# WU-CVGL/Styl3R

Hardware: AMD Instinct MI355X
Metric: 256x256 stylized views/sec (fwd+bwd) @ ~65k Gaussians (higher is better)
Workload: dtype f32; 1 GPU; rasterizer fwd+bwd (decoder API + MSE, the loss computed inside the composite kernels): 10 scenes x 4 target views/GPU/step, 256x256, G=65536 Gaussians/scene (1 ctx view x 256x256), sh_degree=0, make_scale_invariant, all views in one batched launch; outputs the decoder discards are not computed (decoder_splatting_cuda.py:37-68 drops radii / opacity / n_touched, MSE sends no depth gradient: the com; parallelism=dp1 (scenes sharded)

## Files before the change

styl3r_amd/csrc/gsr_common.h:

```cpp
#pragma once
#include <hip/hip_runtime.h>
#include <stdint.h>

#include <type_traits>

#include "../../include/gsr.h"

namespace gsr {

constexpr int TILE = GSR_TILE;
constexpr int TILE_PIX = TILE * TILE;
constexpr int WAVE = 64;

struct alignas(16) SplatRec {
    float x, y, depth;
    uint32_t rad_flags;
    float A, B, C, opacity;
    float r, g, b;
    uint32_t ext;
};
constexpr int LDS_TILES_MAX = 4096;
static_assert(sizeof(SplatRec) == 48, "SplatRec must be 48 bytes");

struct alignas(16) QueueRec {
// ... 46 lines not shown
    return GSR_ELAUNCH;
}
inline bool hip_ok(hipError_t e)
{
    if (e == hipSuccess) return true;
    g_last_hip_error = e;
    return false;
}

struct StageTimer {
    GsrProfile *p; int slot; hipStream_t s;
    StageTimer(void *prof, bool fwd, hipStream_t stream, bool resume = false)
        : p(static_cast<GsrProfile *>(prof)), slot(-1), s(stream)
    {
        if (!p) return;
        int &n = fwd ? p->next_fwd : p->next_bwd;
        if (resume) { if (n > 0 && n <= p->max_calls) slot = n - 1; }
        else if (n < p->max_calls) slot = n++;
    }
    void begin(int stage) { if (slot >= 0 && ((p->mask >> stage) & 1u)) (void)hipEventRecord(p->at(slot, stage, 0), s); }
    void end(int stage) { if (slot >= 0 && ((p->mask >> stage) & 1u)) (void)hipEventRecord(p->at(slot, stage, 1), s); }
};

int layout(const GsrDims &d, long long cap, GsrLayout &L);
Ptrs carve(void *base, const GsrLayout &L);
int forward(const GsrDims &d, const GsrView *views, const float *means, const float *cov6, const float *opac,
            const float *shs, long long cap, void *workspace, size_t workspace_bytes, float *image, float *depth,
            float *opacity, int32_t *radii, int32_t *n_touched, int32_t *status, const GsrFused *fx, hipStream_t stream,
            bool composite = true);
int backward(const GsrDims &d, const GsrView *views, const float *means, const float *cov6, const float *shs,
             long long cap, void *workspace, size_t workspace_bytes, const float *dL_dimage, const float *dL_ddepth,
             float *dL_dmeans, float *dL_dcov6, float *dL_dopac, float *dL_dshs, float *dL_dmeans2D, float *dL_dtau,
             const GsrFused *fx, hipStream_t stream);
int k6_blocks_per_cu(int variant);
int test_reduce9(const float *in, float *out, int rounds, int blocks, int variant, hipStream_t stream);
int forward_styles(const GsrDims &d, int S, const GsrView *views, const float *means, const float *cov6, const float *opac,
                   const float *const *shs, long long cap, void *workspace, size_t workspace_bytes, void *extra, size_t extra_bytes,
                   uint32_t *tile_count, float *image, float *depth, float *opacity, int32_t *radii, int32_t *status, hipStream_t stream);

inline size_t align_up(size_t x, size_t a) { return (x + a - 1) / a * a; }

struct Carver {
    void *base;
    size_t off;
    template <class T>
    T *take(size_t count)
    {
        T *p = base ? reinterpret_cast<T *>(static_cast<char *>(base) + off) : nullptr;
        off += align_up(count * sizeof(T), 256);
        return p;
    }
};

template <class F>
inline void with_sh_degree(const GsrDims &d, F &&f)
{
    switch (d.M > 0 ? d.sh_degree : -1) {
        case -1: f(std::integral_constant<int, -1>{}); break;
        case 0: f(std::integral_constant<int, 0>{}); break;
        case 1: f(std::integral_constant<int, 1>{}); break;
        case 2: f(std::integral_constant<int, 2>{}); break;
        case 3: f(std::integral_constant<int, 3>{}); break;
        default: f(std::integral_constant<int, 4>{}); break;
    }
}

__host__ __device__ inline int tiles_x(int W) { return (W + TILE - 1) / TILE; }
__host__ __device__ inline int tiles_y(int H) { return (H + TILE - 1) / TILE; }

constexpr uint32_t SEG_ONE = 1u << 30;
constexpr int CKPT_SLOT_FLOATS = 5 * TILE_PIX;
__host__ __device__ inline uint32_t seg_len(const GsrDims &d)
{
    switch ((d.flags >> GSR_FLAG_SEG_SHIFT) & 7) {
        case 1: return 64u;
        case 2: return 128u;
        case 3: return 192u;
        case 4: return 256u;
        case 5: return 384u;
        case 7: return SEG_ONE;
        default: {
            const long long vt = (long long)d.B * d.Vt * tiles_x(d.W) * tiles_y(d.H);
            return vt >= 4096 ? 256u : (vt >= 1024 ? 128u : 64u);
        }
    }
}
__host__ __device__ inline size_t unit_capacity(size_t VT, long long cap, uint32_t L) { return VT + (size_t)cap / L; }
__host__ __device__ inline size_t ckpt_slots(long long cap, uint32_t L) { return (size_t)cap / L; }

__device__ constexpr float SH_C0 = 0.28209479177387814f;
__device__ constexpr float SH_C1 = 0.4886025119029199f;
__device__ constexpr float SH_C2_0 = 1.0925484305920792f, SH_C2_1 = -1.0925484305920792f, SH_C2_2 = 0.31539156525252005f,
                           SH_C2_3 = -1.0925484305920792f, SH_C2_4 = 0.5462742152960396f;
__device__ constexpr float SH_C3_0 = -0.5900435899266435f, SH_C3_1 = 2.890611442640554f, SH_C3_2 = -0.4570457994644658f,
                           SH_C3_3 = 0.3731763325901154f, SH_C3_4 = -0.4570457994644658f, SH_C3_5 = 1.445305721320277f,
                           SH_C3_6 = -0.5900435899266435f;
__device__ constexpr float SH_C4_0 = 2.5033429417967046f, SH_C4_1 = -1.7701307697799304f, SH_C4_2 = 0.9461746957575601f,
                           SH_C4_3 = -0.6690465435572892f, SH_C4_4 = 0.10578554691520431f, SH_C4_5 = -0.6690465435572892f,
                           SH_C4_6 = 0.47308734787878004f, SH_C4_7 = -1.7701307697799304f, SH_C4_8 = 0.6258357354491761f;

#pragma clang fp contract(off)

__device__ inline void sh_basis(int deg, float x, float y, float z, float *b)
{
    b[0] = SH_C0;
    if (deg < 1) return;
    b[1] = -SH_C1 * y; b[2] = SH_C1 * z; b[3] = -SH_C1 * x;
    if (deg < 2) return;
    float xx = x * x, yy = y * y, zz = z * z, xy = x * y, yz = y * z, xz = x * z;
    b[4] = SH_C2_0 * xy; b[5] = SH_C2_1 * yz; b[6] = SH_C2_2 * (2.0f * zz - xx - yy);
    b[7] = SH_C2_3 * xz; b[8] = SH_C2_4 * (xx - yy);
    if (deg < 3) return;
    b[9] = SH_C3_0 * y * (3.0f * xx - yy);
    b[10] = SH_C3_1 * xy * z;
    b[11] = SH_C3_2 * y * (4.0f * zz - xx - yy);
    b[12] = SH_C3_3 * z * (2.0f * zz - 3.0f * xx - 3.0f * yy);
    b[13] = SH_C3_4 * x * (4.0f * zz - xx - yy);
    b[14] = SH_C3_5 * z * (xx - yy);
    b[15] = SH_C3_6 * x * (xx - 3.0f * yy);
    if (deg < 4) return;
    b[16] = SH_C4_0 * xy * (xx - yy);
    b[17] = SH_C4_1 * yz * (3.0f * xx - yy);
    b[18] = SH_C4_2 * xy * (7.0f * zz - 1.0f);
    b[19] = SH_C4_3 * yz * (7.0f * zz - 3.0f);
    b[20] = SH_C4_4 * (zz * (35.0f * zz - 30.0f) + 3.0f);
    b[21] = SH_C4_5 * xz * (7.0f * zz - 3.0f);
    b[22] = SH_C4_6 * (xx - yy) * (7.0f * zz - 1.0f);
    b[23] = SH_C4_7 * xz * (xx - 3.0f * yy);
    b[24] = SH_C4_8 * (xx * (xx - 3.0f * yy) - yy * (3.0f * xx - yy));
}

__device__ inline void sh_basis_grad(int deg, float x, float y, float z, float *dx, float *dy, float *dz)
{
    dx[0] = dy[0] = dz[0] = 0.f;
    if (deg < 1) return;
    dx[1] = 0.f; dy[1] = -SH_C1; dz[1] = 0.f;
    dx[2] = 0.f; dy[2] = 0.f; dz[2] = SH_C1;
    dx[3] = -SH_C1; dy[3] = 0.f; dz[3] = 0.f;
    if (deg < 2) return;
    float xx = x * x, yy = y * y, zz = z * z, xy = x * y, yz = y * z, xz = x * z;
    dx[4] = SH_C2_0 * y; dy[4] = SH_C2_0 * x; dz[4] = 0.f;
    dx[5] = 0.f; dy[5] = SH_C2_1 * z; dz[5] = SH_C2_1 * y;
    dx[6] = SH_C2_2 * (-2.0f * x); dy[6] = SH_C2_2 * (-2.0f * y); dz[6] = SH_C2_2 * (4.0f * z);
    dx[7] = SH_C2_3 * z; dy[7] = 0.f; dz[7] = SH_C2_3 * x;
    dx[8] = SH_C2_4 * (2.0f * x); dy[8] = SH_C2_4 * (-2.0f * y); dz[8] = 0.f;
    if (deg < 3) return;
    dx[9] = SH_C3_0 * (6.0f * xy); dy[9] = SH_C3_0 * (3.0f * xx - 3.0f * yy); dz[9] = 0.f;
    dx[10] = SH_C3_1 * yz; dy[10] = SH_C3_1 * xz; dz[10] = SH_C3_1 * xy;
    dx[11] = SH_C3_2 * (-2.0f * xy); dy[11] = SH_C3_2 * (4.0f * zz - xx - 3.0f * yy); dz[11] = SH_C3_2 * (8.0f * yz);
    dx[12] = SH_C3_3 * (-6.0f * xz); dy[12] = SH_C3_3 * (-6.0f * yz); dz[12] = SH_C3_3 * (6.0f * zz - 3.0f * xx - 3.0f * yy);
    dx[13] = SH_C3_4 * (4.0f * zz - 3.0f * xx - yy); dy[13] = SH_C3_4 * (-2.0f * xy); dz[13] = SH_C3_4 * (8.0f * xz);
    dx[14] = SH_C3_5 * (2.0f * xz); dy[14] = SH_C3_5 * (-2.0f * yz); dz[14] = SH_C3_5 * (xx - yy);
    dx[15] = SH_C3_6 * (3.0f * xx - 3.0f * yy); dy[15] = SH_C3_6 * (-6.0f * xy); dz[15] = 0.f;
    if (deg < 4) return;
    dx[16] = SH_C4_0 * y * (3.0f * xx - yy); dy[16] = SH_C4_0 * x * (xx - 3.0f * yy); dz[16] = 0.f;
    dx[17] = SH_C4_1 * (6.0f * xy * z); dy[17] = SH_C4_1 * z * (3.0f * xx - 3.0f * yy); dz[17] = SH_C4_1 * y * (3.0f * xx - yy);
    dx[18] = SH_C4_2 * y * (7.0f * zz - 1.0f); dy[18] = SH_C4_2 * x * (7.0f * zz - 1.0f); dz[18] = SH_C4_2 * (14.0f * xy * z);
    dx[19] = 0.f; dy[19] = SH_C4_3 * z * (7.0f * zz - 3.0f); dz[19] = SH_C4_3 * y * (21.0f * zz - 3.0f);
    dx[20] = 0.f; dy[20] = 0.f; dz[20] = SH_C4_4 * (140.0f * zz * z - 60.0f * z);
    dx[21] = SH_C4_5 * z * (7.0f * zz - 3.0f); dy[21] = 0.f; dz[21] = SH_C4_5 * x * (21.0f * zz - 3.0f);
    dx[22] = SH_C4_6 * (2.0f * x) * (7.0f * zz - 1.0f); dy[22] = SH_C4_6 * (-2.0f * y) * (7.0f * zz - 1.0f); dz[22] = SH_C4_6 * (xx - yy) * (14.0f * z);
    dx[23] = SH_C4_7 * z * (3.0f * xx - 3.0f * yy); dy[23] = SH_C4_7 * (-6.0f * xy * z); dz[23] = SH_C4_7 * x * (xx - 3.0f * yy);
    dx[24] = SH_C4_8 * (4.0f * xx * x - 12.0f * x * yy); dy[24] = SH_C4_8 * (-12.0f * xx * y + 4.0f * yy * y); dz[24] = 0.f;
}

__device__ __forceinline__ void sh_view_dir(const float *m, const float *campos, float &x, float &y, float &z, float &len)
{
    float dx = m[0] - campos[0], dy = m[1] - campos[1], dz = m[2] - campos[2];
    len = sqrtf(dx * dx + dy * dy + dz * dz);
    x = dx / len; y = dy / len; z = dz / len;
}

template <int DEG>
__device__ __forceinline__ uint32_t sh_colour(float x, float y, float z, const float *__restrict__ sh, float *col)
{
    constexpr int NC = (DEG + 1) * (DEG + 1);
    float bs[NC];
    sh_basis(DEG, x, y, z, bs);
    uint32_t clampbits = 0;
#pragma unroll
    for (int c = 0; c < 3; ++c) {
        float acc = bs[0] * sh[c];
#pragma unroll
        for (int k = 1; k < NC; ++k) acc = acc + bs[k] * sh[3 * k + c];
        acc = acc + 0.5f;
        if (acc < 0.f) clampbits |= (1u << c);
        col[c] = fmaxf(acc, 0.f);
    }
    return clampbits;
}

struct Geom {
    float t[3];
    float txc, tyc;
    bool clampx, clampy;
    float J00, J02, J11, J12;
    float M0[3], M1[3];
    float a, b, c;
};

__device__ inline bool geom_eval(const float *V, float tanfovx, float tanfovy, int W, int H, const float *mean,
                                 const float *S, Geom &g)
{
    float px = mean[0], py = mean[1], pz = mean[2];
#pragma unroll
    for (int c = 0; c < 3; ++c) g.t[c] = px * V[0 + c] + py * V[4 + c] + pz * V[8 + c] + V[12 + c];
    if (g.t[2] <= 0.2f) return false;
    float fx = (float)W / (2.0f * tanfovx);
    float fy = (float)H / (2.0f * tanfovy);
    float limx = 1.3f * tanfovx, limy = 1.3f * tanfovy;
    float tz = g.t[2];
    float txtz = g.t[0] / tz, tytz = g.t[1] / tz;
    float cx = fminf(limx, fmaxf(-limx, txtz));
    float cy = fminf(limy, fmaxf(-limy, tytz));
    g.clampx = (txtz < -limx || txtz > limx);
    g.clampy = (tytz < -limy || tytz > limy);
    g.txc = cx * tz;
    g.tyc = cy * tz;
    g.J00 = fx / tz;
    g.J02 = -(fx * g.txc) / (tz * tz);
    g.J11 = fy / tz;
    g.J12 = -(fy * g.tyc) / (tz * tz);
#pragma unroll
    for (int j = 0; j < 3; ++j) {
        float R0 = V[4 * j + 0], R1 = V[4 * j + 1], R2 = V[4 * j + 2];
        g.M0[j] = g.J00 * R0 + g.J02 * R2;
        g.M1[j] = g.J11 * R1 + g.J12 * R2;
    }
    float v0[3], v1[3];
    v0[0] = S[0] * g.M0[0] + S[1] * g.M0[1] + S[2] * g.M0[2];
    v0[1] = S[1] * g.M0[0] + S[3] * g.M0[1] + S[4] * g.M0[2];
    v0[2] = S[2] * g.M0[0] + S[4] * g.M0[1] + S[5] * g.M0[2];
    v1[0] = S[0] * g.M1[0] + S[1] * g.M1[1] + S[2] * g.M1[2];
    v1[1] = S[1] * g.M1[0] + S[3] * g.M1[1] + S[4] * g.M1[2];
    v1[2] = S[2] * g.M1[0] + S[4] * g.M1[1] + S[5] * g.M1[2];
    g.a = (g.M0[0] * v0[0] + g.M0[1] * v0[1] + g.M0[2] * v0[2]) + 0.3f;
    g.b = g.M1[0] * v0[0] + g.M1[1] * v0[1] + g.M1[2] * v0[2];
    g.c = (g.M1[0] * v1[0] + g.M1[1] * v1[1] + g.M1[2] * v1[2]) + 0.3f;
    return true;
}

__device__ inline void load_cov(const float *__restrict__ cov, size_t sg, bool cov9, float *S)
{
    if (cov9) {
        const float *c = cov + 9 * sg;
        S[0] = c[0]; S[1] = c[1]; S[2] = c[2]; S[3] = c[4]; S[4] = c[5]; S[5] = c[8];
    } else {
        const float *c = cov + 6 * sg;
#pragma unroll
        for (int k = 0; k < 6; ++k) S[k] = c[k];
    }
}

__device__ inline int tile_rect(float px, float py, int rad, int gx, int gy, int &minx, int &miny, int &maxx, int &maxy)
{
    minx = min(gx, max(0, (int)((px - (float)rad) / (float)TILE)));
    miny = min(gy, max(0, (int)((py - (float)rad) / (float)TILE)));
    maxx = min(gx, max(0, (int)((px + (float)rad + (float)(TILE - 1)) / (float)TILE)));
    maxy = min(gy, max(0, (int)((py + (float)rad + (float)(TILE - 1)) / (float)TILE)));
    return (maxx - minx) * (maxy - miny);
}

#pragma clang fp contract(fast)

__device__ inline uint32_t quadrant_mask(const float4 q0, const float4 q1, uint32_t ext, int ox, int oy)
{
    uint32_t quad = 0;
    if (ext) {
        const float hx = (float)(ext & 0xffffu), hy = (float)(ext >> 16);
        const float fox = (float)ox - q0.x, foy = (float)oy - q0.y;
        const float A = q1.x, B = q1.y, C = q1.z;
        const float lim = 2.0f * __logf(255.0f * q1.w) * 1.002f + 1e-3f;
#pragma unroll
        for (int k = 0; k < 4; ++k) {
            const float x0 = fox + (float)((k & 1) * 8), x1 = x0 + 7.f;
            const float y0 = foy + (float)((k >> 1) * 8), y1 = y0 + 7.f;
            if (x0 > hx || x1 < -hx || y0 > hy || y1 < -hy) continue;
            float best = 0.f;
            if (!(x0 <= 0.f && x1 >= 0.f && y0 <= 0.f && y1 >= 0.f)) {
                best = 3.0e38f;
                const float iC = -B * __builtin_amdgcn_rcpf(C), iA = -B * __builtin_amdgcn_rcpf(A);
#pragma unroll
                for (int e = 0; e < 2; ++e) {
                    const float xe = e ? x1 : x0;
                    const float dy = fminf(fmaxf(iC * xe, y0), y1);
                    best = fminf(best, A * xe * xe + 2.f * B * xe * dy + C * dy * dy);
                    const float ye = e ? y1 : y0;
                    const float dx = fminf(fmaxf(iA * ye, x0), x1);
                    best = fminf(best, A * dx * dx + 2.f * B * dx * ye + C * ye * ye);
                }
            }
            if (best <= lim) quad |= 1u << k;
        }
    }
    return quad;
}

#define CONIC_PRESCALE 1.4426950408889634f
__device__ inline float footprint_exp(float power) { return __builtin_amdgcn_exp2f(power); }
__device__ inline uint32_t stage_entry_fwd(const SplatRec *__restrict__ recs, uint32_t id, int ox, int oy, float4 *dst)
{
    const float4 *r = reinterpret_cast<const float4 *>(recs + id);
    const float4 q0 = r[0], q1 = r[1], q2 = r[2];
    const uint32_t quad = quadrant_mask(q0, q1, __float_as_uint(q2.w), ox, oy);
    dst[0] = make_float4(q0.x, q0.y, q1.x * CONIC_PRESCALE, q1.y * CONIC_PRESCALE);
    dst[1] = make_float4(q1.z * CONIC_PRESCALE, q1.w, q0.z, __uint_as_float(id));
    dst[2] = make_float4(q2.x, q2.y, q2.z, __uint_as_float(quad));
    return quad;
}
__device__ inline void stage_entry_bwd(const SplatRec *__restrict__ recs, uint32_t id, uint32_t quad, float4 *dst)
{
    const float4 *r = reinterpret_cast<const float4 *>(recs + id);
    const float4 q0 = r[0], q1 = r[1], q2 = r[2];
    dst[0] = make_float4(q0.x, q0.y, q1.x * CONIC_PRESCALE, q1.y * CONIC_PRESCALE);
    dst[1] = make_float4(q1.z * CONIC_PRESCALE, q1.w, q0.z, __uint_as_float(id));
    dst[2] = make_float4(q2.x, q2.y, q2.z, __uint_as_float(quad));
}

__device__ inline float sel_f(unsigned long long m, float t, float f)
{
    float r;
    asm("v_cndmask_b32 %0, %1, %2, %3" : "=v"(r) : "v"(f), "v"(t), "s"(m));
    return r;
}
__device__ inline float sel0_f(unsigned long long m, float t)
{
    float r;
    asm("v_cndmask_b32 %0, 0, %1, %2" : "=v"(r) : "v"(t), "s"(m));
    return r;
}
__device__ inline uint32_t sel_u(unsigned long long m, uint32_t t, uint32_t f)
{
    uint32_t r;
    asm("v_cndmask_b32 %0, %1, %2, %3" : "=v"(r) : "v"(f), "v"(t), "s"(m));
    return r;
}

template <int CTRL, int ROW_MASK = 0xf, int BANK_MASK = 0xf, bool BOUND = false>
__device__ inline float dpp_mov(float v)
{
    return __builtin_bit_cast(float, __builtin_amdgcn_update_dpp(0, __builtin_bit_cast(int, v), CTRL, ROW_MASK, BANK_MASK, BOUND));
}

__device__ inline float wave_sum_to_lane63(float v)
{
    v += dpp_mov<0xb1, 0xf, 0xf, true>(v);
    v += dpp_mov<0x4e, 0xf, 0xf, true>(v);
    v += dpp_mov<0x124, 0xf, 0xf, true>(v);
    v += dpp_mov<0x128, 0xf, 0xf, true>(v);
    v += dpp_mov<0x142, 0xa, 0xf, false>(v);
    v += dpp_mov<0x143, 0xc, 0xf, false>(v);
    return v;
}

__device__ inline double wave_sum(double v)
{
#pragma unroll
    for (int o = 32; o > 0; o >>= 1) v += __shfl_xor(v, o, 64);
    return v;
}

template <bool SLOT>
__device__ inline uint32_t wave_agg_inc(uint32_t *__restrict__ counters, uint32_t t, bool valid)
{
    const int lane = threadIdx.x & 63;
    unsigned long long todo = __ballot(valid);
    int my_leader = lane;
    uint32_t cnt = 0, rank = 0;
    while (todo) {
        const int leader = __ffsll((long long)todo) - 1;
        const uint32_t tl = (uint32_t)__builtin_amdgcn_readlane((int)t, leader);
        const bool mine = valid && t == tl;
        const unsigned long long m = __ballot(mine);
        if (mine) {
            my_leader = leader;
            cnt = (uint32_t)__popcll(m);
            rank = (uint32_t)__popcll(m & ((1ull << lane) - 1ull));
        }
        todo &= ~m;
    }
    uint32_t base = 0;
    if (valid && lane == my_leader) {
        if (SLOT) base = atomicAdd(counters + t, cnt);
        else atomicAdd(counters + t, cnt);
    }
    if (!SLOT) return 0;
    base = (uint32_t)__shfl((int)base, my_leader, 64);
    return base + rank;
}

__device__ inline float row_allsum(float v)
{
    v += dpp_mov<0xb1, 0xf, 0xf, true>(v);
    v += dpp_mov<0x4e, 0xf, 0xf, true>(v);
    v += dpp_mov<0x124, 0xf, 0xf, true>(v);
    v += dpp_mov<0x128, 0xf, 0xf, true>(v);
    return v;
}
__device__ inline float swapsum32(float x, float y)
{
    const auto r = __builtin_amdgcn_permlane32_swap(__float_as_uint(x), __float_as_uint(y), false, false);
    return __uint_as_float(r[0]) + __uint_as_float(r[1]);
}
__device__ inline float swapsum16(float x, float y)
{
    const auto r = __builtin_amdgcn_permlane16_swap(__float_as_uint(x), __float_as_uint(y), false, false);
    return __uint_as_float(r[0]) + __uint_as_float(r[1]);
}
__device__ inline float rows_packed_sum(float x, float y, float u, const bool u_whole_wave)
{
    float z, u8;
    asm volatile("s_nop 1\n\t"
                 "v_add_f32_dpp %0, %2, %2 row_ror:8 row_mask:0xf bank_mask:0x3\n\t"
                 "v_add_f32_dpp %0, %3, %3 row_ror:8 row_mask:0xf bank_mask:0xc\n\t"
                 "v_add_f32_dpp %1, %4, %4 row_ror:8 row_mask:0xf bank_mask:0xf\n\t"
                 "s_nop 0\n\t"
                 "v_add_f32_dpp %0, %0, %0 row_ror:12 row_mask:0xf bank_mask:0x5\n\t"
                 "v_add_f32_dpp %0, %1, %1 row_ror:12 row_mask:0xf bank_mask:0x8\n\t"
                 "s_nop 1\n\t"
                 "v_add_f32_dpp %0, %0, %0 quad_perm:[1,0,3,2] row_mask:0xf bank_mask:0xf\n\t"
                 "s_nop 1\n\t"
                 "v_add_f32_dpp %0, %0, %0 quad_perm:[2,3,0,1] row_mask:0xf bank_mask:0xf"
                 : "=&v"(z), "=&v"(u8) : "v"(x), "v"(y), "v"(u));
    if (u_whole_wave)
        asm volatile("s_nop 1\n\t"
                     "v_add_f32_dpp %0, %0, %0 row_bcast:15 row_mask:0xa bank_mask:0x8\n\t"
                     "s_nop 1\n\t"
                     "v_add_f32_dpp %0, %0, %0 row_bcast:31 row_mask:0xc bank_mask:0x8" : "+v"(z));
    return z;
}
__device__ inline float wave_reduce10(const float *a)
{
    const float b0 = swapsum32(a[0], a[5]), b1 = swapsum32(a[1], a[6]), b2 = swapsum32(a[2], a[7]), b3 = swapsum32(a[3], a[8]),
                b4 = swapsum32(a[4], a[9]);
    return rows_packed_sum(swapsum16(b0, b1), swapsum16(b2, b3), swapsum16(b4, 0.f), false);
}
__device__ inline int reduce10_slot(int lane)
{
    const int r = lane >> 4, s = lane & 15;
    if (s == 0) return (r < 2) ? r : r + 3;
    if (s == 8) return (r < 2) ? r + 2 : r + 5;
    if (s == 12) return (r == 0) ? 4 : (r == 2 ? 9 : -1);
    return -1;
}
__device__ inline float wave_reduce9(const float *v)
{
    const float b0 = swapsum32(v[0], v[4]), b1 = swapsum32(v[1], v[5]), b2 = swapsum32(v[2], v[6]), b3 = swapsum32(v[3], v[7]);
    return rows_packed_sum(swapsum16(b0, b1), swapsum16(b2, b3), v[8], true);
}
__device__ inline int reduce9_slot(int lane)
{
    const int r = lane >> 4, s = lane & 15;
    if (s == 0) return (r < 2) ? r : r + 2;
    if (s == 8) return (r < 2) ? r + 2 : r + 4;
    return lane == 63 ? 8 : -1;
}
__device__ inline float wave_reduce9_lds(const float *v, float *s_red, int lane)
{
#pragma unroll
    for (int i = 0; i < 8; ++i) s_red[i * 64 + lane] = v[i];
    asm volatile("" ::: "memory");
    const float4 p = reinterpret_cast<const float4 *>(s_red)[lane], q = reinterpret_cast<const float4 *>(s_red)[64 + lane];
    asm volatile("" ::: "memory");
    return rows_packed_sum((p.x + p.y) + (p.z + p.w), (q.x + q.y) + (q.z + q.w), v[8], true);
}
__device__ inline int reduce9_lds_slot(int lane)
{
    const int r = lane >> 4, s = lane & 15;
    if (s == 0) return r;
    if (s == 8) return r + 4;
    return lane == 63 ? 8 : -1;
}

}
```

styl3r_amd/csrc/gsr_forward.hip:

```cpp
#include <cstdlib>
#include <cstring>
#include <type_traits>

#include "gsr_common.h"

namespace gsr {

#pragma clang fp contract(off)
template <int DEG>
__global__ void __launch_bounds__(256) k_preprocess(GsrDims d, const GsrView *__restrict__ views,
                                                    const float *__restrict__ means, const float *__restrict__ cov6,
                                                    const float *__restrict__ opac, const float *__restrict__ shs,
                                                    Ptrs ws, int32_t *__restrict__ radii, int lds_tiles)
{
    extern __shared__ uint32_t s_tiles[];
    const int g = blockIdx.x * blockDim.x + threadIdx.x;
    const int b = blockIdx.y;
    const bool live = g < d.G;
    const size_t sg = (size_t)b * d.G + (live ? g : 0);
    const float m0[3] = {means[3 * sg], means[3 * sg + 1], means[3 * sg + 2]};
    float S0[6];
    load_cov(cov6, sg, (d.flags & GSR_FLAG_COV9) != 0, S0);
    const float op = opac[sg];
    if (live) ws.opac[sg] = op;
// ... 265 lines not shown
    }
    uint32_t ftotal;
    const uint32_t fpos = t.full_base + block_excl_scan_256<uint32_t>(unit ? nf : 0u, s4, ftotal);
    if (i >= n) return;
    ws.tile_order[s_base[cls] + atomicAdd(&s_cnt[cls], 1u)] = (uint32_t)i;
    if (!unit) return;
    for (uint32_t s = 0; s < nf; ++s)
        if (fpos + s < umax) ws.unit_order[fpos + s] = make_uint2((uint32_t)i, s);
    const uint32_t p = t.full + s_base[ucl] + atomicAdd(&s_cnt[ucl], 1u);
    if (p < umax) ws.unit_order[p] = make_uint2((uint32_t)i, nf);
}

#pragma clang fp contract(off)
__global__ void __launch_bounds__(256) k_scatter(GsrDims d, Ptrs ws)
{
    if (ws.status[GSR_ST_OVERFLOW]) return;
    const int g = blockIdx.x * blockDim.x + threadIdx.x;
    const int v = blockIdx.y;
    const bool live = g < d.G;
    const size_t vg = (size_t)v * d.G + (live ? g : 0);
    const float4 q0 = ws.geo[vg];
    const int rad = live ? (int)(__float_as_uint(q0.w) & 0xffffffu) : 0;
    const int gx = tiles_x(d.W), gy = tiles_y(d.H), T = gx * gy;
    int minx = 0, miny = 0, maxx = 0, maxy = 0;
    if (rad > 0) tile_rect(q0.x, q0.y, rad, gx, gy, minx, miny, maxx, maxy);
    const unsigned long long key = ((unsigned long long)__float_as_uint(q0.z) << 32) | (unsigned)g;
    const size_t tb = (size_t)v * T;
    const int rw = maxx - minx, area = rw * (maxy - miny);
    int amax = area;
#pragma unroll
    for (int o = 32; o > 0; o >>= 1) amax = max(amax, __shfl_xor(amax, o, 64));
    for (int k = 0; k < amax; ++k) {
        const bool has = k < area;
        const int ty = has ? miny + k / rw : 0, tx = has ? minx + k % rw : 0;
        const uint32_t tl = (uint32_t)(ty * gx + tx);
        const uint32_t slot = wave_agg_inc<true>(ws.tile_cursor + tb, tl, has);
        if (has) ws.pairs[ws.tile_offset[tb + tl] + slot] = key;
    }
}
#pragma clang fp contract(fast)

__global__ void __launch_bounds__(256) k_scatter_lds(GsrDims d, Ptrs ws)
{
    if (ws.status[GSR_ST_OVERFLOW]) return;
    extern __shared__ uint32_t s_sc[];
    const int g = blockIdx.x * blockDim.x + threadIdx.x;
    const int v = blockIdx.y;
    const bool live = g < d.G;
    const size_t vg = (size_t)v * d.G + (live ? g : 0);
    const float4 q0 = ws.geo[vg];
    const int rad = live ? (int)(__float_as_uint(q0.w) & 0xffffffu) : 0;
    const int gx = tiles_x(d.W), gy = tiles_y(d.H), T = gx * gy;
    uint32_t *s_cnt = s_sc, *s_base = s_sc + T;
    for (int t = threadIdx.x; t < T; t += 256) s_cnt[t] = 0u;
    int minx = 0, miny = 0, maxx = 0, maxy = 0;
    if (rad > 0) tile_rect(q0.x, q0.y, rad, gx, gy, minx, miny, maxx, maxy);
    const unsigned long long key = ((unsigned long long)__float_as_uint(q0.z) << 32) | (unsigned)g;
    const size_t tb = (size_t)v * T;
    const int rw = maxx - minx, area = rw * (maxy - miny);
    __syncthreads();
    for (int k = 0; k < area; ++k) atomicAdd(&s_cnt[(miny + k / rw) * gx + minx + k % rw], 1u);
    __syncthreads();
    for (int t = threadIdx.x; t < T; t += 256) {
        const uint32_t c = s_cnt[t];
        if (c) { s_base[t] = ws.tile_offset[tb + t] + atomicAdd(ws.tile_cursor + tb + t, c); s_cnt[t] = 0u; }
    }
    __syncthreads();
    for (int k = 0; k < area; ++k) {
        const int tl = (miny + k / rw) * gx + minx + k % rw;
        ws.pairs[s_base[tl] + atomicAdd(&s_cnt[tl], 1u)] = key;
    }
}

template <typename KeyPtr>
__device__ inline void bitonic_sort_block(KeyPtr key, uint32_t n, int tid, int nthreads)
{
    uint32_t N = 1;
    while (N < n) N <<= 1;
    for (uint32_t k = 2; k <= N; k <<= 1) {
        {
            const uint32_t half = k >> 1;
            for (uint32_t p = tid; p < (N >> 1); p += nthreads) {
                uint32_t blk = p / half, q = p - blk * half;
                uint32_t i = blk * k + q, l = blk * k + (k - 1 - q);
                if (l < n) {
                    unsigned long long a = key[i], c = key[l];
                    if (a > c) { key[i] = c; key[l] = a; }
                }
            }
            __syncthreads();
        }
        for (uint32_t j = k >> 2; j > 0; j >>= 1) {
            for (uint32_t p = tid; p < (N >> 1); p += nthreads) {
                uint32_t i = ((p & ~(j - 1)) << 1) | (p & (j - 1));
                uint32_t l = i | j;
                if (l < n) {
                    unsigned long long a = key[i], c = key[l];
                    if (a > c) { key[i] = c; key[l] = a; }
                }
            }
            __syncthreads();
        }
    }
}

__device__ inline void ce(unsigned long long &a, unsigned long long &b, bool asc)
{
    const bool sw = asc ? (a > b) : (a < b);
    const unsigned long long t = sw ? b : a;
    b = sw ? a : b; a = t;
}
__device__ inline void bitonic_sort_1024(unsigned long long *s, uint32_t n, int tid)
{
    uint32_t N = 4;
    while (N < n) N <<= 1;
    for (uint32_t i = n + tid; i < N; i += 256) s[i] = ~0ull;
    __syncthreads();
    const uint32_t G = N >> 2;
    if ((uint32_t)tid < G) {
        const uint32_t i = (uint32_t)tid << 2;
        unsigned long long e0 = s[i], e1 = s[i + 1], e2 = s[i + 2], e3 = s[i + 3];
        ce(e0, e1, true); ce(e2, e3, false);
        const bool asc = (i & 4u) == 0;
        ce(e0, e2, asc); ce(e1, e3, asc); ce(e0, e1, asc); ce(e2, e3, asc);
        s[i] = e0; s[i + 1] = e1; s[i + 2] = e2; s[i + 3] = e3;
    }
    __syncthreads();
    for (uint32_t k = 8; k <= N; k <<= 1) {
        uint32_t j = k >> 1;
        for (; j >= 2; j >>= 2) {
            if ((uint32_t)tid < G) {
                const uint32_t h = j >> 1, g = (uint32_t)tid;
                const uint32_t i0 = (g / h) * (j << 1) + (g % h);
                const bool asc = (i0 & k) == 0;
                unsigned long long e0 = s[i0], e1 = s[i0 + h], e2 = s[i0 + j], e3 = s[i0 + j + h];
                ce(e0, e2, asc); ce(e1, e3, asc); ce(e0, e1, asc); ce(e2, e3, asc);
                s[i0] = e0; s[i0 + h] = e1; s[i0 + j] = e2; s[i0 + j + h] = e3;
            }
            __syncthreads();
        }
        if (j == 1) {
            for (uint32_t p = tid; p < (N >> 1); p += 256) {
                const uint32_t i = p << 1;
                unsigned long long a = s[i], b = s[i + 1];
                ce(a, b, (i & k) == 0);
                s[i] = a; s[i + 1] = b;
            }
            __syncthreads();
        }
    }
}

constexpr uint32_t SORT_LDS_KEYS = 4096;

constexpr uint32_t RADIX_BINS = 256, RANK_MAX = 128;

__device__ inline uint32_t radix_digit(unsigned long long key, uint32_t dmin, uint32_t shift)
{
    return ((uint32_t)(key >> 32) - dmin) >> shift;
}

struct TileOut {
    uint32_t *point_list;
    __device__ void put(uint32_t pos, unsigned long long key) const { point_list[pos] = (uint32_t)(key & 0xffffffffull); }
};

__device__ inline void rank_and_emit(unsigned long long *s_key, uint32_t m, uint32_t b0, uint32_t b1, const uint32_t *s_start,
                                     const uint32_t *s_big, uint32_t nbig, uint32_t dmin, uint32_t shift, const TileOut &out, int tid)
{
    const uint32_t base = s_start[b0];
    for (uint32_t p = tid; p < m; p += 256) {
        const unsigned long long key = s_key[p];
        const uint32_t dg = radix_digit(key, dmin, shift);
        const uint32_t s0 = s_start[dg] - base, s1 = s_start[dg + 1] - base;
        if (s1 - s0 > RANK_MAX) continue;
        uint32_t rank = s0;
        for (uint32_t q = s0; q < s1; ++q) rank += (s_key[q] < key) ? 1u : 0u;
        out.put(base + rank, key);
    }
    for (uint32_t b = 0; b < nbig; ++b) {
        const uint32_t dg = s_big[b];
        if (dg < b0 || dg >= b1) continue;
        const uint32_t s0 = s_start[dg] - base, cnt = s_start[dg + 1] - s_start[dg];
        __syncthreads();
        bitonic_sort_block(s_key + s0, cnt, tid, 256);
        for (uint32_t i = tid; i < cnt; i += 256) out.put(base + s0 + i, s_key[s0 + i]);
    }
    __syncthreads();
}

__global__ void __launch_bounds__(256) k_tile_sort(GsrDims d, Ptrs ws, uint32_t lds_keys)
{
    if (ws.status[GSR_ST_OVERFLOW]) return;
    extern __shared__ unsigned long long s_key[];
    __shared__ uint32_t s_hist[RADIX_BINS], s_start[RADIX_BINS + 1], s_big[RADIX_BINS];
    __shared__ uint32_t s_red[12], s_nbig;
    const int gx = tiles_x(d.W), T = gx * tiles_y(d.H);
    const uint32_t tv = ws.tile_order[blockIdx.y * gridDim.x + blockIdx.x];
    const int tile = (int)(tv % (uint32_t)T), v = (int)(tv / (uint32_t)T);
    const size_t t = (size_t)v * T + tile;
    const uint32_t start = ws.tile_offset[t];
    const uint32_t n = ws.tile_offset[t + 1] - start;
    if (n == 0) return;
    const int tid = threadIdx.x, lane = tid & 63, wid = tid >> 6;
    TileOut out;
    out.point_list = ws.point_list + start;
    const unsigned long long *gk = ws.pairs + start;
    if (n <= 64) {
        for (uint32_t i = tid; i < n; i += 256) s_key[i] = gk[i];
        __syncthreads();
        if (n > 1) bitonic_sort_1024(s_key, n, tid);
        for (uint32_t i = tid; i < n; i += 256) out.put(i, s_key[i]);
        return;
    }
    const bool in_regs = n <= 1024u;
    unsigned long long kreg[4] = {0ull, 0ull, 0ull, 0ull};
    if (in_regs) {
#pragma unroll
        for (int e = 0; e < 4; ++e) { const uint32_t i = tid + 256u * e; if (i < n) kreg[e] = gk[i]; }
    }
    auto for_my_keys = [&](auto fn) {
        if (in_regs) {
#pragma unroll
            for (int e = 0; e < 4; ++e) if (tid + 256u * e < n) fn(kreg[e]);
        } else {
            for (uint32_t i = tid; i < n; i += 256) fn(gk[i]);
        }
    };
    uint32_t mn = 0xffffffffu, mx = 0u;
    for_my_keys([&](unsigned long long key) { const uint32_t dep = (uint32_t)(key >> 32); mn = min(mn, dep); mx = max(mx, dep); });
    s_hist[tid] = 0u;
    if (tid == 0) s_nbig = 0u;
#pragma unroll
    for (int o = 32; o > 0; o >>= 1) {
        mn = min(mn, (uint32_t)__shfl_xor((int)mn, o, 64));
        mx = max(mx, (uint32_t)__shfl_xor((int)mx, o, 64));
    }
    if (lane == 0) { s_red[wid] = mn; s_red[4 + wid] = mx; }
    __syncthreads();
    const uint32_t dmin = min(min(s_red[0], s_red[1]), min(s_red[2], s_red[3]));
    const uint32_t dmax = max(max(s_red[4], s_red[5]), max(s_red[6], s_red[7]));
    const uint32_t range = dmax - dmin;
    const uint32_t nbits = range ? 32u - (uint32_t)__clz((int)range) : 0u;
    const uint32_t shift = nbits > 8u ? nbits - 8u : 0u;
    for_my_keys([&](unsigned long long key) { atomicAdd(&s_hist[radix_digit(key, dmin, shift)], 1u); });
    __syncthreads();
    {
        const uint32_t c = s_hist[tid];
        uint32_t x = c;
#pragma unroll
        for (int o = 1; o < 64; o <<= 1) {
            const uint32_t y = (uint32_t)__shfl_up((int)x, o, 64);
            if (lane >= o) x += y;
        }
        if (lane == 63) s_red[8 + wid] = x;
        __syncthreads();
        uint32_t off = x - c;
        for (int w = 0; w < wid; ++w) off += s_red[8 + w];
        s_start[tid] = off;
        if (tid == 255) s_start[256] = off + c;
        if (c > RANK_MAX) s_big[atomicAdd(&s_nbig, 1u)] = (uint32_t)tid;
        s_hist[tid] = 0u;
    }
    __syncthreads();
    const uint32_t nbig = s_nbig;
    if (n <= lds_keys) {
        for_my_keys([&](unsigned long long key) {
            const uint32_t dg = radix_digit(key, dmin, shift);
            s_key[s_start[dg] + atomicAdd(&s_hist[dg], 1u)] = key;
        });
        __syncthreads();
        rank_and_emit(s_key, n, 0u, RADIX_BINS, s_start, s_big, nbig, dmin, shift, out, tid);
        return;
    }
    unsigned long long *alt = ws.pairs_alt + start;
    for (uint32_t i = tid; i < n; i += 256) {
        const unsigned long long key = gk[i];
        const uint32_t dg = radix_digit(key, dmin, shift);
        alt[s_start[dg] + atomicAdd(&s_hist[dg], 1u)] = key;
    }
    __syncthreads();
    uint32_t b0 = 0;
    while (b0 < RADIX_BINS) {
        uint32_t b1 = b0 + 1;
        while (b1 < RADIX_BINS && s_start[b1 + 1] - s_start[b0] <= lds_keys) ++b1;
        const uint32_t base = s_start[b0], m = s_start[b1] - base;
        if (m > lds_keys) {
            bitonic_sort_block(alt + base, m, tid, 256);
            for (uint32_t i = tid; i < m; i += 256) out.put(base + i, alt[base + i]);
            __syncthreads();
        } else if (m > 0) {
            for (uint32_t i = tid; i < m; i += 256) s_key[i] = alt[base + i];
            __syncthreads();
            rank_and_emit(s_key, m, b0, b1, s_start, s_big, nbig, dmin, shift, out, tid);
        }
        b0 = b1;
    }
}

__device__ inline void agent_publish(float *p, float v)
{
    (void)__hip_atomic_exchange(reinterpret_cast<uint32_t *>(p), __float_as_uint(v), __ATOMIC_RELAXED, __HIP_MEMORY_SCOPE_AGENT);
}
__device__ inline float agent_read(float *p)
{
    return __uint_as_float(__hip_atomic_fetch_or(reinterpret_cast<uint32_t *>(p), 0u, __ATOMIC_RELAXED, __HIP_MEMORY_SCOPE_AGENT));
}

template <bool NTOUCH>
__global__ void __launch_bounds__(64) k_composite_fwd(GsrDims d, const GsrView *__restrict__ views, Ptrs ws,
                                                     float *__restrict__ image, float *__restrict__ out_depth,
                                                     float *__restrict__ out_opacity, int32_t *__restrict__ n_touched,
                                                     const float *__restrict__ mse_target, float mse_weight,
                                                     float *__restrict__ mse_loss)
{
    if (ws.status[GSR_ST_OVERFLOW]) return;
    __shared__ float4 s_q[64 * 3];

    const int gx = tiles_x(d.W), T = gx * tiles_y(d.H);
    const uint32_t tv = ws.tile_order[blockIdx.y * gridDim.x + blockIdx.x];
    const int tile = (int)(tv % (uint32_t)T), v = (int)(tv / (uint32_t)T);
    const int lane = threadIdx.x;
    const int ox = (tile % gx) * TILE + (lane & 7), oy = (tile / gx) * TILE + (lane >> 3);

    if (d.flags & GSR_FLAG_PREZERO_GRADS) {
        const size_t n4 = (size_t)d.B * d.Vt * d.G * (GR_STRIDE / 4);
        const size_t nwg = (size_t)gridDim.x * gridDim.y, wg = (size_t)blockIdx.y * gridDim.x + blockIdx.x;
        const size_t per = (n4 + nwg - 1) / nwg, lo = wg * per, hi = lo + per < n4 ? lo + per : n4;
        float4 *gz = reinterpret_cast<float4 *>(ws.grad_rec);
        for (size_t i = lo + lane; i < hi; i += 64) gz[i] = make_float4(0.f, 0.f, 0.f, 0.f);
    }

    const size_t t = (size_t)v * T + tile;
    const uint32_t start = ws.tile_offset[t];
    const int n = (int)(ws.tile_offset[t + 1] - start);
    uint32_t *__restrict__ plist = ws.point_list + start;
    const SplatRec *__restrict__ recs = ws.records + (size_t)v * d.G;
    const int tile_ox = (tile % gx) * TILE, tile_oy = (tile / gx) * TILE;

    float fx0 = (float)ox, fy0 = (float)oy;
    asm volatile("" : "+v"(fx0), "+v"(fy0));
    float Tr[4], C0[4], C1[4], C2[4], D[4], O[4];
    uint32_t last[4];
    bool inside[4];
    unsigned long long dmask[4];
#pragma unroll
    for (int k = 0; k < 4; ++k) {
        const int px = ox + (k & 1) * 8, py = oy + (k >> 1) * 8;
        inside[k] = px < d.W && py < d.H;
        Tr[k] = 1.f; C0[k] = C1[k] = C2[k] = D[k] = O[k] = 0.f;
        last[k] = 0;
        dmask[k] = __builtin_amdgcn_ballot_w64(!inside[k]);
    }
    const uint32_t seg = seg_len(d);
    uint32_t ck_next = seg, ck_slot = start / seg;

    for (int base = 0; base < n; base += 64) {
        const int cnt = __builtin_amdgcn_readfirstlane(min(64, n - base));
        __syncthreads();
        uint32_t qm = 0;
        if (lane < cnt) {
            const uint32_t id = plist[base + lane] & GSR_ID_MASK;
            qm = stage_entry_fwd(recs, id, tile_ox, tile_oy, s_q + lane * 3);
            if (qm) plist[base + lane] = id | (qm << GSR_QUAD_SHIFT);
        }
        __syncthreads();

        for (unsigned long long todo = __builtin_amdgcn_ballot_w64(qm != 0u); todo; todo &= todo - 1ull) {
            const int j = __builtin_ctzll(todo);
            const float4 a = s_q[j * 3 + 0];
            const float4 b = s_q[j * 3 + 1];
            const float4 c = s_q[j * 3 + 2];
            const uint32_t quad = __builtin_amdgcn_readfirstlane(__float_as_uint(c.w));
            uint32_t touched_tot = 0;
#pragma unroll
            for (int k = 0; k < 4; ++k) {
                if (!(quad & (1u << k))) continue;
                if (dmask[k] == ~0ull) continue;
                const float dx = (a.x - fx0) - (float)((k & 1) * 8), dy = (a.y - fy0) - (float)((k >> 1) * 8);
                const float power = -0.5f * (a.z * dx * dx + b.x * dy * dy) - a.w * dx * dy;
                const float alpha = fminf(0.99f, b.y * footprint_exp(power));
                const float test_T = Tr[k] * (1.f - alpha);
                const unsigned long long live = __builtin_amdgcn_ballot_w64(!(power > 0.f)) & __builtin_amdgcn_ballot_w64(!(alpha < (1.f / 255.f))) & ~dmask[k];
                const unsigned long long keep = __builtin_amdgcn_ballot_w64(!(test_T < 0.0001f));
                dmask[k] |= live & ~keep;
                const unsigned long long comp = live & keep;
                const float w = sel0_f(comp, alpha * Tr[k]);
                C0[k] += c.x * w; C1[k] += c.y * w; C2[k] += c.z * w;
                D[k] += b.z * w;
                O[k] += w;
                if (NTOUCH) touched_tot += (uint32_t)__popcll(comp & __builtin_amdgcn_ballot_w64(test_T > 0.5f));
                Tr[k] = sel_f(comp, test_T, Tr[k]);
                last[k] = sel_u(comp, (uint32_t)(base + j + 1), last[k]);
            }
            if (NTOUCH) {
                if (touched_tot && lane == 0) atomicAdd(n_touched + (size_t)v * d.G + (__float_as_uint(b.w)), (int)touched_tot);
            }
        }
        if ((uint32_t)(base + 64) == ck_next && ck_next < (uint32_t)n) {
            float *slot = ws.ckpt + (size_t)ck_slot * CKPT_SLOT_FLOATS;
#pragma unroll
            for (int k = 0; k < 4; ++k) {
                reinterpret_cast<float4 *>(slot)[k * 64 + lane] = make_float4(Tr[k], C0[k], C1[k], C2[k]);
                slot[4 * TILE_PIX + k * 64 + lane] = D[k];
            }
            ck_next += seg; ++ck_slot;
        }
        if ((dmask[0] & dmask[1] & dmask[2] & dmask[3]) == ~0ull) break;
    }

    const size_t P = (size_t)d.H * d.W;
    const GsrView &vw = views[v];
    float sq = 0.f;
#pragma unroll
    for (int k = 0; k < 4; ++k) {
        if (!inside[k]) continue;
        const size_t pix = (size_t)(oy + (k >> 1) * 8) * d.W + (ox + (k & 1) * 8);
        ws.final_T[v * P + pix] = Tr[k];
        ws.n_contrib[v * P + pix] = last[k];
        const float r0 = C0[k] + Tr[k] * vw.bg[0], r1 = C1[k] + Tr[k] * vw.bg[1], r2 = C2[k] + Tr[k] * vw.bg[2];
        image[(v * 3 + 0) * P + pix] = r0;
        image[(v * 3 + 1) * P + pix] = r1;
        image[(v * 3 + 2) * P + pix] = r2;
        out_depth[v * P + pix] = D[k];
        out_opacity[v * P + pix] = O[k];
        if ((uint32_t)n > seg) ws.final_C[v * P + pix] = make_float4(C0[k], C1[k], C2[k], D[k]);
        if (mse_target) {
            const float e0 = r0 - mse_target[(v * 3 + 0) * P + pix], e1 = r1 - mse_target[(v * 3 + 1) * P + pix],
                        e2 = r2 - mse_target[(v * 3 + 2) * P + pix];
            sq += (e0 * e0 + e1 * e1) + e2 * e2;
            ws.loss_diff[(v * 3 + 0) * P + pix] = e0; ws.loss_diff[(v * 3 + 1) * P + pix] = e1; ws.loss_diff[(v * 3 + 2) * P + pix] = e2;
        }
    }
    if (!mse_target) return;
    const int V = d.B * d.Vt;
    sq = wave_sum_to_lane63(sq);
    uint32_t arrived = 0;
    if (lane == 63) {
        agent_publish(ws.loss_partial + t, sq);
        asm volatile("s_waitcnt vmcnt(0)" ::: "memory");
        arrived = __hip_atomic_fetch_add(ws.loss_ticket + v, 1u, __ATOMIC_RELAXED, __HIP_MEMORY_SCOPE_AGENT);
    }
    arrived = (uint32_t)__builtin_amdgcn_readlane((int)arrived, 63);
    if (arrived != (uint32_t)T - 1u) return;
    float s1 = 0.f;
    for (int i = lane; i < T; i += 64) s1 += agent_read(ws.loss_partial + (size_t)v * T + i);
    s1 = wave_sum_to_lane63(s1);
    arrived = 0;
    if (lane == 63) {
        agent_publish(ws.loss_partial + (size_t)V * T + v, s1);
        asm volatile("s_waitcnt vmcnt(0)" ::: "memory");
        arrived = __hip_atomic_fetch_add(ws.loss_ticket + V, 1u, __ATOMIC_RELAXED, __HIP_MEMORY_SCOPE_AGENT);
    }
    arrived = (uint32_t)__builtin_amdgcn_readlane((int)arrived, 63);
    if (arrived != (uint32_t)V - 1u) return;
    float s2 = 0.f;
    for (int i = lane; i < V; i += 64) s2 += agent_read(ws.loss_partial + (size_t)V * T + i);
    s2 = wave_sum_to_lane63(s2);
    if (lane == 63) mse_loss[0] = mse_weight * (s2 / (float)((size_t)V * 3 * P));
}

int layout(const GsrDims &d, long long cap, GsrLayout &L)
{
    if (d.B <= 0 || d.Vt <= 0 || d.G <= 0 || d.H <= 0 || d.W <= 0 || cap <= 0) return GSR_EINVAL;
    if (d.M < 0 || d.sh_degree < 0 || d.sh_degree > 4) return GSR_EINVAL;
    if (d.M > 0 && (d.sh_degree + 1) * (d.sh_degree + 1) > d.M) return GSR_EINVAL;
    if (d.M == 0 && d.sh_degree != 0) return GSR_EINVAL;
    if (cap > 0xffffffffll) return GSR_EINVAL;
    if ((long long)d.G * (long long)sizeof(SplatRec) > 0xffffffffll) return GSR_EINVAL;
    static_assert((0xffffffffull / sizeof(SplatRec)) < GSR_ID_MASK, "ids must leave the quadrant-mask bits of a point_list word free");
    const size_t V = (size_t)d.B * d.Vt, T = (size_t)tiles_x(d.W) * tiles_y(d.H), P = (size_t)d.H * d.W;
    size_t off = 0;
    auto take = [&](size_t bytes) { size_t o = off; off = align_up(off + bytes, 256); return o; };
    L.records = take(V * d.G * sizeof(SplatRec));
    L.tile_count = take(V * T * 4);
    L.tile_offset = take((V * T + 1) * 4);
    L.tile_cursor = take(V * T * 4);
    L.pairs = take((size_t)cap * 8);
    L.point_list = take((size_t)cap * 4);
    L.final_T = take(V * P * 4);
    L.n_contrib = take(V * P * 4);
    L.grad_rec = take(V * d.G * 12 * 4);
    L.status = take(GSR_STATUS_WORDS * 4);
    L.tile_order = take(V * T * 4);
    L.pairs_alt = take((size_t)cap * 8);
    L.loss_partial = take((V * T + V) * 4);
    L.loss_ticket = take((V + 1) * 4);
    L.loss_diff = take(V * 3 * P * 4);
    const uint32_t seg = seg_len(d);
    L.final_C = take(seg == SEG_ONE ? 0 : V * P * 16);
    L.ckpt = take(ckpt_slots(cap, seg) * CKPT_SLOT_FLOATS * 4);
    L.unit_order = take(unit_capacity(V * T, cap, seg) * 8);
    L.geo = take(V * d.G * 16);
    L.opac = take((size_t)d.B * d.G * 4);
    L.scan = take(scan_words(V * T) * 4);
    L.total = off;
    return GSR_OK;
}

Ptrs carve(void *base, const GsrLayout &L)
{
    char *p = static_cast<char *>(base);
    Ptrs w;
    w.records = reinterpret_cast<SplatRec *>(p + L.records);
    w.tile_count = reinterpret_cast<uint32_t *>(p + L.tile_count);
    w.tile_offset = reinterpret_cast<uint32_t *>(p + L.tile_offset);
    w.tile_cursor = reinterpret_cast<uint32_t *>(p + L.tile_cursor);
    w.pairs = reinterpret_cast<unsigned long long *>(p + L.pairs);
    w.point_list = reinterpret_cast<uint32_t *>(p + L.point_list);
    w.final_T = reinterpret_cast<float *>(p + L.final_T);
    w.n_contrib = reinterpret_cast<uint32_t *>(p + L.n_contrib);
    w.grad_rec = reinterpret_cast<float *>(p + L.grad_rec);
    w.status = reinterpret_cast<int32_t *>(p + L.status);
    w.tile_order = reinterpret_cast<uint32_t *>(p + L.tile_order);
    w.pairs_alt = reinterpret_cast<unsigned long long *>(p + L.pairs_alt);
    w.loss_partial = reinterpret_cast<float *>(p + L.loss_partial);
    w.loss_ticket = reinterpret_cast<uint32_t *>(p + L.loss_ticket);
    w.loss_diff = reinterpret_cast<float *>(p + L.loss_diff);
    w.final_C = reinterpret_cast<float4 *>(p + L.final_C);
    w.ckpt = reinterpret_cast<float *>(p + L.ckpt);
    w.unit_order = reinterpret_cast<uint2 *>(p + L.unit_order);
    w.geo = reinterpret_cast<float4 *>(p + L.geo);
    w.opac = reinterpret_cast<float *>(p + L.opac);
    w.scan = reinterpret_cast<uint32_t *>(p + L.scan);
    return w;
}

int forward(const GsrDims &d, const GsrView *views, const float *means, const float *cov6, const float *opac,
            const float *shs, long long cap, void *workspace, size_t workspace_bytes, float *image, float *depth,
            float *opacity, int32_t *radii, int32_t *n_touched, int32_t *status, const GsrFused *fx, hipStream_t stream,
            bool composite)
{
    GsrLayout L;
    int rc = layout(d, cap, L);
    if (rc != GSR_OK) return rc;
    if (!views || !means || !cov6 || !opac || !shs || !workspace || !image || !depth || !opacity || !radii || !status)
        return GSR_EINVAL;
    const bool ntouch = (d.flags & GSR_FLAG_NTOUCHED) != 0;
    if (ntouch && !n_touched) return GSR_EINVAL;
    if (workspace_bytes < L.total) return GSR_ENOSPACE;
    const float *mse_target = fx ? fx->mse_target : nullptr;
    if (mse_target && !fx->mse_loss) return GSR_EINVAL;
    Ptrs ws = carve(workspace, L);
    const bool persistent_counters = fx && fx->tile_count;
    if (persistent_counters) ws.tile_count = fx->tile_count;
    const int V = d.B * d.Vt, gx = tiles_x(d.W), gy = tiles_y(d.H), T = gx * gy;
    (void)hipGetLastError();
    const bool bin = (d.flags & GSR_FLAG_PHASE_BIN) != 0, render = (d.flags & GSR_FLAG_PHASE_RENDER) != 0;
    if (bin && render) return GSR_EINVAL;
    StageTimer tm(d.profile, true, stream, render);
    const dim3 gG((d.G + 255) / 256, d.B), gV((d.G + 255) / 256, V);
    const int lds_tiles = (T <= LDS_TILES_MAX && !(d.flags & GSR_FLAG_BIN_BALLOT)) ? T : 0;
    if (render) goto render_phase;

    if (!persistent_counters && !hip_ok(hipMemsetAsync(ws.tile_count, 0, (size_t)V * T * 4, stream))) return GSR_ELAUNCH;
    if (ntouch && !hip_ok(hipMemsetAsync(n_touched, 0, (size_t)V * d.G * 4, stream))) return GSR_ELAUNCH;

    tm.begin(GSR_STAGE_PREPROCESS);
    with_sh_degree(d, [&](auto deg) {
        hipLaunchKernelGGL(k_preprocess<decltype(deg)::value>, gG, dim3(256), lds_tiles * 4, stream, d, views, means, cov6, opac, shs, ws, radii, lds_tiles);
    });
    tm.end(GSR_STAGE_PREPROCESS); tm.begin(GSR_STAGE_SCAN);
    {
        const uint32_t seg = seg_len(d);
        const int n = V * T;
        const dim3 gS((n + SCAN_CHUNK - 1) / SCAN_CHUNK);
        hipLaunchKernelGGL(k_scan_partials, gS, dim3(SCAN_CHUNK), 0, stream, n, ws, mse_target ? V + 1 : 0, seg);
        hipLaunchKernelGGL(k_scan_offsets, gS, dim3(SCAN_CHUNK), 0, stream, n, cap, ws, status, seg);
        hipLaunchKernelGGL(k_scan_place, gS, dim3(SCAN_CHUNK), 0, stream, n, cap, ws, persistent_counters ? 1 : 0, seg,
                           (uint32_t)unit_capacity((size_t)V * T, cap, seg));
    }
    tm.end(GSR_STAGE_SCAN);
    if (bin) return launch_status();
render_phase:
    tm.begin(GSR_STAGE_SCATTER);
    if (lds_tiles) hipLaunchKernelGGL(k_scatter_lds, gV, dim3(256), lds_tiles * 8, stream, d, ws);
    else hipLaunchKernelGGL(k_scatter, gV, dim3(256), 0, stream, d, ws);
    tm.end(GSR_STAGE_SCATTER); tm.begin(GSR_STAGE_SORT);
    {
        const int sel = (d.flags >> GSR_FLAG_SORT_KEYS_SHIFT) & 3;
        const uint32_t lds_keys = sel == 1 ? 1024u : (sel == 2 ? 2048u : SORT_LDS_KEYS);
        hipLaunchKernelGGL(k_tile_sort, dim3(T, V), dim3(256), lds_keys * 8, stream, d, ws, lds_keys);
    }
    tm.end(GSR_STAGE_SORT);
    if (!composite) return launch_status();
    tm.begin(GSR_STAGE_COMPOSITE_FWD);
    {
        const float mse_weight = fx ? fx->mse_weight : 0.f;
        float *mse_loss = fx ? fx->mse_loss : nullptr;
        if (ntouch) hipLaunchKernelGGL(k_composite_fwd<true>, dim3(T, V), dim3(64), 0, stream, d, views, ws, image, depth, opacity, n_touched, mse_target, mse_weight, mse_loss);
        else hipLaunchKernelGGL(k_composite_fwd<false>, dim3(T, V), dim3(64), 0, stream, d, views, ws, image, depth, opacity, n_touched, mse_target, mse_weight, mse_loss);
    }
    tm.end(GSR_STAGE_COMPOSITE_FWD);
    return launch_status();
}

}
```

Measured before the change: 31340 views/s.

## Interleave gradient prezeroing stores with forward composite batches

Instead of zeroing each workgroup's slice of the gradient buffer up front, the forward composite kernel now issues one 64-wide zeroing store per staged batch of splats and drains any remainder after the loss reduction. The goal is to hide the zeroing stores behind the compositing math rather than delaying the start of rasterization. It also reorders the staging writes so the quadrant mask is computed after the first LDS stores, uses uniform scalar offsets, and moves the MSE ticket reduction into a helper. This adds per-batch bookkeeping and leaves the remainder zeroing on the kernel's tail, which could lengthen tiles with few splats.

New measurement: 31490 views/s (median of 6 runs). Within noise of the previous version (+0.5%).

```diff
diff --git a/styl3r_amd/csrc/gsr_common.h b/styl3r_amd/csrc/gsr_common.h
--- a/styl3r_amd/csrc/gsr_common.h
+++ b/styl3r_amd/csrc/gsr_common.h
@@ -372,10 +372,11 @@
 {
     const float4 *r = reinterpret_cast<const float4 *>(recs + id);
     const float4 q0 = r[0], q1 = r[1], q2 = r[2];
-    const uint32_t quad = quadrant_mask(q0, q1, __float_as_uint(q2.w), ox, oy);
     dst[0] = make_float4(q0.x, q0.y, q1.x * CONIC_PRESCALE, q1.y * CONIC_PRESCALE);
     dst[1] = make_float4(q1.z * CONIC_PRESCALE, q1.w, q0.z, __uint_as_float(id));
-    dst[2] = make_float4(q2.x, q2.y, q2.z, __uint_as_float(quad));
+    dst[2] = make_float4(q2.x, q2.y, q2.z, 0.f);
+    const uint32_t quad = quadrant_mask(q0, q1, __float_as_uint(q2.w), ox, oy);
+    reinterpret_cast<uint32_t *>(dst + 2)[3] = quad;
     return quad;
 }
 __device__ inline void stage_entry_bwd(const SplatRec *__restrict__ recs, uint32_t id, uint32_t quad, float4 *dst)
diff --git a/styl3r_amd/csrc/gsr_forward.hip b/styl3r_amd/csrc/gsr_forward.hip
--- a/styl3r_amd/csrc/gsr_forward.hip
+++ b/styl3r_amd/csrc/gsr_forward.hip
@@ -591,9 +591,51 @@
 {
     (void)__hip_atomic_exchange(reinterpret_cast<uint32_t *>(p), __float_as_uint(v), __ATOMIC_RELAXED, __HIP_MEMORY_SCOPE_AGENT);
 }
+__device__ inline size_t uniform_u64(size_t x)
+{
+    return ((size_t)(uint32_t)__builtin_amdgcn_readfirstlane((int)(x >> 32)) << 32) | (uint32_t)__builtin_amdgcn_readfirstlane((int)x);
+}
+__device__ inline void zero_piece(float4 *&zp, uint32_t &left, int lane)
+{
+    float z = 0.f;
+    uint32_t l = (uint32_t)lane;
+    asm volatile("" : "+v"(z), "+v"(l));
+    if (l < left) *reinterpret_cast<float4 *>(reinterpret_cast<char *>(zp) + l * 16u) = make_float4(z, z, z, z);
+    zp += 64;
+    left = left > 64u ? left - 64u : 0u;
+}
 __device__ inline float agent_read(float *p)
 {
     return __uint_as_float(__hip_atomic_fetch_or(reinterpret_cast<uint32_t *>(p), 0u, __ATOMIC_RELAXED, __HIP_MEMORY_SCOPE_AGENT));
+}
+
+__device__ inline void fused_mse_arrive(const Ptrs &ws, size_t t, int v, int T, int V, size_t P, int lane, float sq, float mse_weight,
+                                        float *__restrict__ mse_loss)
+{
+    sq = wave_sum_to_lane63(sq);
+    uint32_t arrived = 0;
+    if (lane == 63) {
+        agent_publish(ws.loss_partial + t, sq);
+        asm volatile("s_waitcnt vmcnt(0)" ::: "memory");
+        arrived = __hip_atomic_fetch_add(ws.loss_ticket + v, 1u, __ATOMIC_RELAXED, __HIP_MEMORY_SCOPE_AGENT);
+    }
+    arrived = (uint32_t)__builtin_amdgcn_readlane((int)arrived, 63);
+    if (arrived != (uint32_t)T - 1u) return;
+    float s1 = 0.f;
+    for (int i = lane; i < T; i += 64) s1 += agent_read(ws.loss_partial + (size_t)v * T + i);
+    s1 = wave_sum_to_lane63(s1);
+    arrived = 0;
+    if (lane == 63) {
+        agent_publish(ws.loss_partial + (size_t)V * T + v, s1);
+        asm volatile("s_waitcnt vmcnt(0)" ::: "memory");
+        arrived = __hip_atomic_fetch_add(ws.loss_ticket + V, 1u, __ATOMIC_RELAXED, __HIP_MEMORY_SCOPE_AGENT);
+    }
+    arrived = (uint32_t)__builtin_amdgcn_readlane((int)arrived, 63);
+    if (arrived != (uint32_t)V - 1u) return;
+    float s2 = 0.f;
+    for (int i = lane; i < V; i += 64) s2 += agent_read(ws.loss_partial + (size_t)V * T + i);
+    s2 = wave_sum_to_lane63(s2);
+    if (lane == 63) mse_loss[0] = mse_weight * (s2 / (float)((size_t)V * 3 * P));
 }
 
 template <bool NTOUCH>
@@ -612,12 +654,16 @@
     const int lane = threadIdx.x;
     const int ox = (tile % gx) * TILE + (lane & 7), oy = (tile / gx) * TILE + (lane >> 3);
 
+    float4 *zp = reinterpret_cast<float4 *>(ws.grad_rec);
+    uint32_t zleft = 0;
     if (d.flags & GSR_FLAG_PREZERO_GRADS) {
         const size_t n4 = (size_t)d.B * d.Vt * d.G * (GR_STRIDE / 4);
         const size_t nwg = (size_t)gridDim.x * gridDim.y, wg = (size_t)blockIdx.y * gridDim.x + blockIdx.x;
         const size_t per = (n4 + nwg - 1) / nwg, lo = wg * per, hi = lo + per < n4 ? lo + per : n4;
-        float4 *gz = reinterpret_cast<float4 *>(ws.grad_rec);
-        for (size_t i = lo + lane; i < hi; i += 64) gz[i] = make_float4(0.f, 0.f, 0.f, 0.f);
+        if (lo < hi) {
+            zp += uniform_u64(lo);
+            zleft = (uint32_t)__builtin_amdgcn_readfirstlane((int)(uint32_t)(hi - lo));
+        }
     }
 
     const size_t t = (size_t)v * T + tile;
@@ -651,9 +697,14 @@
         if (lane < cnt) {
             const uint32_t id = plist[base + lane] & GSR_ID_MASK;
             qm = stage_entry_fwd(recs, id, tile_ox, tile_oy, s_q + lane * 3);
-            if (qm) plist[base + lane] = id | (qm << GSR_QUAD_SHIFT);
+            if (qm) {
+                uint32_t l = (uint32_t)lane;
+                asm volatile("" : "+v"(l));
+                *reinterpret_cast<uint32_t *>(reinterpret_cast<char *>(plist + base) + l * 4u) = id | (qm << GSR_QUAD_SHIFT);
+            }
         }
         __syncthreads();
+        zero_piece(zp, zleft, lane);
 
         for (unsigned long long todo = __builtin_amdgcn_ballot_w64(qm != 0u); todo; todo &= todo - 1ull) {
             const int j = __builtin_ctzll(todo);
@@ -721,32 +772,8 @@
             ws.loss_diff[(v * 3 + 0) * P + pix] = e0; ws.loss_diff[(v * 3 + 1) * P + pix] = e1; ws.loss_diff[(v * 3 + 2) * P + pix] = e2;
         }
     }
-    if (!mse_target) return;
-    const int V = d.B * d.Vt;
-    sq = wave_sum_to_lane63(sq);
-    uint32_t arrived = 0;
-    if (lane == 63) {
-        agent_publish(ws.loss_partial + t, sq);
-        asm volatile("s_waitcnt vmcnt(0)" ::: "memory");
-        arrived = __hip_atomic_fetch_add(ws.loss_ticket + v, 1u, __ATOMIC_RELAXED, __HIP_MEMORY_SCOPE_AGENT);
-    }
-    arrived = (uint32_t)__builtin_amdgcn_readlane((int)arrived, 63);
-    if (arrived != (uint32_t)T - 1u) return;
-    float s1 = 0.f;
-    for (int i = lane; i < T; i += 64) s1 += agent_read(ws.loss_partial + (size_t)v * T + i);
-    s1 = wave_sum_to_lane63(s1);
-    arrived = 0;
-    if (lane == 63) {
-        agent_publish(ws.loss_partial + (size_t)V * T + v, s1);
-        asm volatile("s_waitcnt vmcnt(0)" ::: "memory");
-        arrived = __hip_atomic_fetch_add(ws.loss_ticket + V, 1u, __ATOMIC_RELAXED, __HIP_MEMORY_SCOPE_AGENT);
-    }
-    arrived = (uint32_t)__builtin_amdgcn_readlane((int)arrived, 63);
-    if (arrived != (uint32_t)V - 1u) return;
-    float s2 = 0.f;
-    for (int i = lane; i < V; i += 64) s2 += agent_read(ws.loss_partial + (size_t)V * T + i);
-    s2 = wave_sum_to_lane63(s2);
-    if (lane == 63) mse_loss[0] = mse_weight * (s2 / (float)((size_t)V * 3 * P));
+    if (mse_target) fused_mse_arrive(ws, t, v, T, d.B * d.Vt, P, lane, sq, mse_weight, mse_loss);
+    while (zleft) zero_piece(zp, zleft, lane);
 }
 
 int layout(const GsrDims &d, long long cap, GsrLayout &L)
```
